# HIRO-group/torque_constrained_motion_planning

Measured on AMD Instinct MI355X. Metric: torque-feasible collision-checked RRT* samples/sec, Panda 7-DOF, 1/2/4/8 GPU, higher is better.
Workload: dtype f64

## Files before the change

include/tcmp.h:

```cpp
#ifndef TCMP_H_
#define TCMP_H_

#include <stdint.h>

#ifdef __cplusplus
extern "C" {
#endif

typedef struct tcmp_handle tcmp_handle;
typedef struct tcmp_comm tcmp_comm;

#define TCMP_TORQUE_BASE 0
#define TCMP_TORQUE_NOV 1
#define TCMP_TORQUE_RNE 2
#define TCMP_TORQUE_DYN 3

#define TCMP_PLAN_OK 0
#define TCMP_PLAN_START_GOAL_COLLISION 1
#define TCMP_PLAN_NO_GOAL 2
#define TCMP_PLAN_VALIDATION_FAILED 3
#define TCMP_PLAN_MINJERK_ASSERT 4

int tcmp_create(int device, tcmp_handle** out);
int tcmp_destroy(tcmp_handle* h);
// ... 43 lines not shown

int tcmp_check_configs(tcmp_handle* h, const double* q, int64_t n, int32_t* collides);

int tcmp_check_body(tcmp_handle* h, const double* q, int64_t n, int32_t* collides);

int tcmp_base_pd(tcmp_handle* h, double* pd, int32_t n);

enum {
  TCMP_PD_CHAIN = 0, TCMP_PD_BOX32 = 1, TCMP_PD_BOX64 = 2, TCMP_PD_HULL32 = 3, TCMP_PD_HULL64 = 4,
  TCMP_PD_LOD_IN = 5, TCMP_PD_LOD_OUT = 6, TCMP_PD_FACET_AXES = 7, TCMP_PD_SPHERE_CERT = 8
};
enum { TCMP_PD_NO_PRUNE = 1, TCMP_PD_INNER_BOX = 2 };
int tcmp_debug_pair_pd(tcmp_handle* h, const int32_t* link, const double* pose,
                       const int32_t* obstacle, int64_t n, int32_t stage, int32_t flags,
                       double* pd, int32_t* info);

int tcmp_gauss_clusters(const tcmp_hulls* H, int32_t n, double* records, float* cones,
                        int32_t* cluster_off);

int tcmp_check_edges(tcmp_handle* h, const double* from, const double* to, int64_t n,
                     const double* resolutions, int32_t torque_mode, double payload_mass,
                     int32_t* n_safe, int32_t* n_steps, double* last);

typedef struct {
  int32_t max_anchors;
  int32_t passes;
} tcmp_shortcut_cfg;

typedef struct {
  int32_t status;
// ... 150 lines not shown
```

torque_constrained_motion_planning_amd/_lib.py:

```python
import ctypes
import os
import threading

import numpy as np

HERE = os.path.dirname(os.path.abspath(__file__))
LIB_PATH = os.environ.get("TCMP_LIB_PATH", os.path.join(HERE, "libtcmp.so"))

_dp = ctypes.POINTER(ctypes.c_double)
_i32p = ctypes.POINTER(ctypes.c_int32)
_i64p = ctypes.POINTER(ctypes.c_int64)
_u8p = ctypes.POINTER(ctypes.c_uint8)

TORQUE_BASE, TORQUE_NOV, TORQUE_RNE, TORQUE_DYN = 0, 1, 2, 3
PLAN_OK, PLAN_START_GOAL_COLLISION, PLAN_NO_GOAL, PLAN_VALIDATION_FAILED, PLAN_MINJERK_ASSERT = range(5)

EXPORTS = [
    "tcmp_create", "tcmp_destroy", "tcmp_last_error", "tcmp_device_count", "tcmp_version",
    "tcmp_synchronize",
    "tcmp_set_scene", "tcmp_set_meshes", "tcmp_set_mesh_lods", "tcmp_set_mesh_spheres", "tcmp_set_self_collision", "tcmp_set_timing", "tcmp_rne_batch", "tcmp_torque_ok", "tcmp_check_configs",
    "tcmp_check_body", "tcmp_base_pd",
    "tcmp_check_edges", "tcmp_nearest", "tcmp_minjerk", "tcmp_validate_traj",
    "tcmp_plan_begin", "tcmp_plan_round", "tcmp_plan_goal", "tcmp_plan_run", "tcmp_plan_finish",
    "tcmp_plan_retrace",
    "tcmp_plan_run_shared", "tcmp_plan_run_group", "tcmp_plan_run_fused", "tcmp_plan_begin_many",
    "tcmp_plan_finish_many",
    "tcmp_plan_fetch", "tcmp_plan_tree", "tcmp_plan_digest", "tcmp_plan_debug_round", "tcmp_ik", "tcmp_fk",
    "tcmp_debug_counters", "tcmp_microbench",
    "tcmp_rendezvous", "tcmp_dist_init", "tcmp_dist_destroy", "tcmp_dist_rank",
    "tcmp_dist_barrier", "tcmp_dist_allreduce", "tcmp_dist_allgather_i64", "tcmp_gather_paths",
    "tcmp_gather_layout", "tcmp_gather_pack", "tcmp_gather_unpack", "tcmp_dist_rccl_ranks",
    "tcmp_shortcut_path", "tcmp_plan_shortcut",
    "tcmp_tier0_tables", "tcmp_tier0_masks",
    "tcmp_debug_pair_pd", "tcmp_gauss_clusters",
]
(PD_CHAIN, PD_BOX32, PD_BOX64, PD_HULL32, PD_HULL64, PD_LOD_IN, PD_LOD_OUT, PD_FACET_AXES,
 PD_SPHERE_CERT) = range(9)
PD_NO_PRUNE, PD_INNER_BOX = 1, 2
TRAJ_COLS = 22
REDUCE_SUM, REDUCE_MAX = 0, 1


class PlanCfg(ctypes.Structure):
    _fields_ = [
        ("start", ctypes.c_double * 7), ("goal", ctypes.c_double * 7),
        ("weights", ctypes.c_double * 7), ("resolutions", ctypes.c_double * 7),
        ("radius", ctypes.c_double), ("goal_probability", ctypes.c_double),
        ("goal_tolerance", ctypes.c_double), ("payload_mass", ctypes.c_double),
        ("execution_time", ctypes.c_double), ("seed", ctypes.c_uint64),
# ... 138 lines not shown
        if hasattr(L, "tcmp_shortcut_path"):
            L.tcmp_shortcut_path.argtypes = [vp, _dp, ctypes.c_int64, _dp, _dp, ctypes.c_int32,
                                             ctypes.c_double, ctypes.POINTER(ShortcutCfg), _dp,
                                             ctypes.c_int64, ctypes.POINTER(ShortcutResult)]
            L.tcmp_plan_shortcut.argtypes = [vp, ctypes.POINTER(ShortcutCfg),
                                             ctypes.POINTER(ShortcutResult)]
        if hasattr(L, "tcmp_tier0_tables"):
            _f32p, _u32p = ctypes.POINTER(ctypes.c_float), ctypes.POINTER(ctypes.c_uint32)
            L.tcmp_tier0_tables.argtypes = [_dp, ctypes.c_int32, ctypes.c_int32, _f32p, _u32p, _f32p]
            L.tcmp_tier0_masks.argtypes = [_u32p, ctypes.c_int32, _f32p, _f32p, ctypes.c_int64, _u32p]
        if hasattr(L, "tcmp_debug_pair_pd"):
            L.tcmp_debug_pair_pd.argtypes = [vp, _i32p, _dp, _i32p, ctypes.c_int64, ctypes.c_int32,
                                             ctypes.c_int32, _dp, _i32p]
            L.tcmp_gauss_clusters.argtypes = [ctypes.POINTER(Hulls), ctypes.c_int32, _dp,
                                              ctypes.POINTER(ctypes.c_float), _i32p]
        _lib = L
        return L


def _d(a):
    return None if a is None else a.ctypes.data_as(_dp)


def _rows(x, name="array"):
    a = np.ascontiguousarray(np.asarray(x, dtype=np.float64))
    if a.ndim == 1:
        a = a.reshape(1, -1)
    if a.shape[-1] != 7:
        raise ValueError("%s must have 7 columns, got shape %s" % (name, a.shape))
    return a.reshape(-1, 7)
# ... 146 lines not shown
        self._check(self.L.tcmp_base_pd(self.h, _d(out) if n else None, n))
        return out

    def debug_pair_pd(self, link, pose, obstacle, stage, flags=0):
        pose = np.ascontiguousarray(np.asarray(pose, dtype=np.float64).reshape(-1, 12))
        n = len(pose)
        link = np.ascontiguousarray(np.broadcast_to(np.asarray(link, dtype=np.int32), (n,)))
        obstacle = np.ascontiguousarray(np.broadcast_to(np.asarray(obstacle, dtype=np.int32), (n,)))
        pd = np.zeros(n)
        info = np.zeros(n, dtype=np.int32)
        self._check(self.L.tcmp_debug_pair_pd(self.h, link.ctypes.data_as(_i32p), _d(pose),
                                              obstacle.ctypes.data_as(_i32p), n, int(stage),
                                              int(flags), _d(pd), info.ctypes.data_as(_i32p)))
        return pd, info

    def check_edges(self, q_from, q_to, mode, mass, resolutions=None):
        a = _rows(q_from, "from"); b = _rows(q_to, "to")
        n = len(a)
        ns = np.zeros(n, dtype=np.int32); nt = np.zeros(n, dtype=np.int32)
        last = np.zeros((n, 7))
        res = None if resolutions is None else np.ascontiguousarray(resolutions, dtype=np.float64)
        self._check(self.L.tcmp_check_edges(self.h, _d(a), _d(b), n, _d(res), int(mode),
                                            float(mass), ns.ctypes.data_as(_i32p),
                                            nt.ctypes.data_as(_i32p), _d(last)))
        return ns, nt, last

    def shortcut_path(self, waypoints, torque_mode, payload_mass, resolutions=None, weights=None,
                      max_anchors=512, passes=1):
        if not hasattr(self.L, "tcmp_shortcut_path"):
            raise TcmpError("tcmp_shortcut_path: not in this library build")
# ... 341 lines not shown
```

torque_constrained_motion_planning_amd/csrc/tcmp_device.h:

```cpp
#pragma once
#include <hip/hip_runtime.h>
#include <stdint.h>

#define TCMP_GEO_QUAL static constexpr
#include "panda_geometry.inc"
#include "panda_lod.inc"
#include "panda_spheres.inc"

namespace tcmp {

constexpr double kPen = 0.04;

constexpr double kLo[7] = {-2.8973, -1.7628, -2.8973, -3.0718, -2.8973, -0.0175, -2.8973};
constexpr double kHi[7] = {2.8973, 1.7628, 2.8973, -0.0698, 2.8973, 3.7525, 2.8973};
constexpr double kEffort[7] = {87.0, 87.0, 87.0, 87.0, 12.0, 12.0, 12.0};

constexpr double kC90 = 6.123233995736766e-17;
constexpr double kDhA[8] = {0.0, 0.0, 0.0, 0.0825, -0.0825, 0.0, 0.088, 0.0};
constexpr double kDhD[8] = {0.333, 0.0, 0.316, 0.0, 0.384, 0.0, 0.0, 0.107};
constexpr double kDhCa[8] = {1.0, kC90, kC90, kC90, kC90, kC90, kC90, 1.0};
constexpr double kDhSa[8] = {0.0, -1.0, 1.0, 1.0, -1.0, 1.0, 1.0, 0.0};

constexpr double kMass[7] = {4.970684, 0.646926, 3.228604, 3.587895, 1.225946, 1.666555,
                             7.35522e-01};
// ... 509 lines not shown
            m0 = -m0; m1 = -m1; m2 = -m2;
          }
          const double hv = m0 * va.x + m1 * va.y + m2 * va.z;
          const double pc = m0 * cl[0] + m1 * cl[1] + m2 * cl[2];
          const double rad = h[0] * fabs(m0 * A[0] + m1 * A[3] + m2 * A[6]) +
                             h[1] * fabs(m0 * A[1] + m1 * A[4] + m2 * A[7]) +
                             h[2] * fabs(m0 * A[2] + m1 * A[5] + m2 * A[8]);
          loc = fmin(loc, (hv - pc + rad) / sqrt(len2));
        }
      }
    }
  }
  return fmin(pd, wave_min(loc));
}

__device__ __forceinline__ float wave_minf(float x) {
  x = fminf(x, dpp_f<0xB1>(x));
  x = fminf(x, dpp_f<0x4E>(x));
  x = fminf(x, dpp_f<0x124>(x));
  x = fminf(x, dpp_f<0x128>(x));
  x = fminf(x, bc15_f(x));
  x = fminf(x, bc31_f(x));
  return readlane_f(x, 63);
}
__device__ __forceinline__ float wave_minf_bc(float x) {
  x = fminf(x, dpp_f<0xB1>(x));
  x = fminf(x, dpp_f<0x4E>(x));
  x = fminf(x, dpp_f<0x124>(x));
  x = fminf(x, dpp_f<0x128>(x));
  x = fminf(x, bc15_f(x));
  x = fminf(x, bc31_f(x));
  return readlane_f(x, 63);
}
__device__ __forceinline__ float wave_maxf(float x) {
  x = fmaxf(x, dpp_f<0xB1>(x));
  x = fmaxf(x, dpp_f<0x4E>(x));
  x = fmaxf(x, dpp_f<0x124>(x));
  x = fmaxf(x, dpp_f<0x128>(x));
  x = fmaxf(x, bc15_f(x));
  x = fmaxf(x, bc31_f(x));
  return readlane_f(x, 63);
}

constexpr float kExactGuard = 1e-4f;
constexpr int max_link_edges() {
  int m = 0;
  for (int l = 0; l < TCMP_NLINKS; ++l) {
    const int n = tcmp_geo_edge_off[l + 1] - tcmp_geo_edge_off[l];
    m = n > m ? n : m;
  }
  return m;
}
#ifdef TCMP_PROF_EXACT
__device__ unsigned long long g_fa_hist[32];
__device__ unsigned long long g_sb_hist[32];
__device__ unsigned long long g_pass_stats[8];
__device__ unsigned long long g_exact_stats[32];
#endif
__device__ __forceinline__ float exact_pd_wave32(int link, const Pose pose,
                                              const double* __restrict__ ob, const Geo g,
                                              bool box_pair = false) {
  const int lane = lane_id();
#ifdef TCMP_PROF_EXACT
  unsigned long long tb = clock64();
#define TCMP_BOX_CLK(i) if (box_pair) { const unsigned long long t1 = clock64(); \
    if (lane == 0) atomicAdd(&g_exact_stats[16 + (i)], t1 - tb); tb = t1; }
#else
#define TCMP_BOX_CLK(i)
#endif
  const double* R = pose.R;
  const double* p = pose.p;
  const double d[3] = {ob[0] - p[0], ob[1] - p[1], ob[2] - p[2]};
  float cl[3], A[9];
#pragma unroll
  for (int i = 0; i < 3; ++i) {
    cl[i] = (float)(R[0 + i] * d[0] + R[3 + i] * d[1] + R[6 + i] * d[2]);
// ... 5 lines not shown
  constexpr float P = (float)kPen;
  const int v0 = tcmp_geo_vert_off[link], v1 = tcmp_geo_vert_off[link + 1];
  const int f0 = tcmp_geo_plane_off[link], f1 = tcmp_geo_plane_off[link + 1];
  const int e0 = tcmp_geo_edge_off[link], e1 = tcmp_geo_edge_off[link + 1];
  float mn0 = INFINITY, mn1 = INFINITY, mn2 = INFINITY;
  float mx0 = -INFINITY, mx1 = -INFINITY, mx2 = -INFINITY;
  for (int v = v0 + lane; v < v1; v += 64) {
    const float x = g.verts32[3 * v], y = g.verts32[3 * v + 1], z = g.verts32[3 * v + 2];
    const float d0 = A[0] * x + A[3] * y + A[6] * z;
    const float d1 = A[1] * x + A[4] * y + A[7] * z;
    const float d2 = A[2] * x + A[5] * y + A[8] * z;
    mn0 = fminf(mn0, d0); mx0 = fmaxf(mx0, d0);
    mn1 = fminf(mn1, d1); mx1 = fmaxf(mx1, d1);
    mn2 = fminf(mn2, d2); mx2 = fmaxf(mx2, d2);
  }
  mn0 = wave_minf(mn0); mn1 = wave_minf(mn1); mn2 = wave_minf(mn2);
  mx0 = wave_maxf(mx0); mx1 = wave_maxf(mx1); mx2 = wave_maxf(mx2);
  float pd;
  {
    const float pc0 = A[0] * cl[0] + A[3] * cl[1] + A[6] * cl[2];
    const float pc1 = A[1] * cl[0] + A[4] * cl[1] + A[7] * cl[2];
    const float pc2 = A[2] * cl[0] + A[5] * cl[1] + A[8] * cl[2];
    pd = fminf(fminf(mx0 - pc0 + h[0], pc0 + h[0] - mn0),
               fminf(fminf(mx1 - pc1 + h[1], pc1 + h[1] - mn1),
                     fminf(mx2 - pc2 + h[2], pc2 + h[2] - mn2)));
  }
  TCMP_BOX_CLK(0);
  if (pd < P - kExactGuard) {
#ifdef TCMP_PROF_EXACT
    if (lane == 0) atomicAdd(&g_exact_stats[0], 1ull);
#endif
    return pd;
  }
  TCMP_BOX_CLK(1);
  float loc = INFINITY;
  for (int f = f0 + lane; f < f1; f += 64) {
    const float4 n = g.planes32[f];
    const float pc = n.x * cl[0] + n.y * cl[1] + n.z * cl[2];
    const float rad = h[0] * fabsf(n.x * A[0] + n.y * A[3] + n.z * A[6]) +
                      h[1] * fabsf(n.x * A[1] + n.y * A[4] + n.z * A[7]) +
                      h[2] * fabsf(n.x * A[2] + n.y * A[5] + n.z * A[8]);
    loc = fminf(loc, n.w - pc + rad);
  }
  {
    const float lf = fminf(pd, wave_minf(loc));
    TCMP_BOX_CLK(2);
    if (lf < P - kExactGuard) {
#ifdef TCMP_PROF_EXACT
      if (lane == 0) atomicAdd(&g_exact_stats[1], 1ull);
#endif
      return lf;
    }
  }
  static_assert(max_link_edges() <= 640, "pass-1 marks: 3 bits per 64-edge slice in 32");
  bool deg = false;
  unsigned sil = 0;
  for (int it = 0, base = e0; base < e1; ++it, base += 64) {
    const int e = base + lane;
    if (e < e1) {
      const ushort4 ix = g.eidx[e];
// ... 46 lines not shown
        deg = true;
      } else {
        const float ori = m0 * (n1.x + n2.x) + m1 * (n1.y + n2.y) + m2 * (n1.z + n2.z);
        const float il = rsqrtf(len2);
        deg |= fabsf(ori) * il < 1e-4f;
        if (ori < 0.f) { m0 = -m0; m1 = -m1; m2 = -m2; }
        const float hv = m0 * ax0 + m1 * ay0 + m2 * az0;
        const float pc = m0 * cl[0] + m1 * cl[1] + m2 * cl[2];
        const float rad = h[0] * fabsf(m0 * A[0] + m1 * A[3] + m2 * A[6]) +
                          h[1] * fabsf(m0 * A[1] + m1 * A[4] + m2 * A[7]) +
                          h[2] * fabsf(m0 * A[2] + m1 * A[5] + m2 * A[8]);
        loc = fminf(loc, (hv - pc + rad) * il);
      }
    }
    if (w0 + 64 < total && !__ballot(deg)) {
      const float lf = fminf(pd, wave_minf(loc));
      if (lf < P - kExactGuard) {
#ifdef TCMP_PROF_EXACT
        if (lane == 0) atomicAdd(&g_exact_stats[2], 1ull);
        if (lane == 0 && box_pair) atomicAdd(&g_exact_stats[27], 1ull);
#endif
        return lf;
      }
    }
  }
#ifdef TCMP_PROF_EXACT
  if (lane == 0) atomicAdd(&g_exact_stats[__ballot(deg) ? 3 : 2], 1ull);
#endif
  if (__ballot(deg)) return __builtin_nanf("");
  const float full = fminf(pd, wave_minf(loc));
#ifdef TCMP_PROF_EXACT
  if (lane == 0 && box_pair) atomicAdd(&g_exact_stats[full >= P ? 28 : 29], 1ull);
#endif
  TCMP_BOX_CLK(3);
  return full;
#undef TCMP_BOX_CLK
}

}
#include "tcmp_mesh.h"
namespace tcmp {

__device__ __forceinline__ float facet_axes_wave(int link, const float R[9], const float p[3], int mi,
                                                 const int* rg, const Scene sc, const Geo g) {
  const int lane = lane_id();
  const float4* LS = sc.csph + TCMP_NSPH * link;
  const float4* MS = sc.sph + TCMP_NSPH * (TCMP_NLINKS + mi);
  float best = -INFINITY, bx = 1.f, by = 0.f, bz = 0.f;
#pragma unroll
  for (int k = lane; k < TCMP_NSPH * TCMP_NSPH; k += 64) {
    const float4 t = MS[k % TCMP_NSPH];
    const float4 s = LS[k / TCMP_NSPH];
    const float dx = t.x - p[0], dy = t.y - p[1], dz = t.z - p[2];
    const float ex = R[0] * dx + R[3] * dy + R[6] * dz - s.x;
    const float ey = R[1] * dx + R[4] * dy + R[7] * dz - s.y;
    const float ez = R[2] * dx + R[5] * dy + R[8] * dz - s.z;
    const float ov = s.w + t.w - __builtin_sqrtf(ex * ex + ey * ey + ez * ez);
    if (ov > best) { best = ov; bx = ex; by = ey; bz = ez; }
  }
  {
    const float m = wave_maxf(best);
    const int L = __builtin_ctzll(__ballot(best == m));
    bx = __shfl(bx, L); by = __shfl(by, L); bz = __shfl(bz, L);
    const float l2 = bx * bx + by * by + bz * bz;
    if (!(l2 > 1e-12f)) return INFINITY;
    const float il = rsqrtf(l2);
    bx *= il; by *= il; bz *= il;
  }
  const float ax = R[0] * bx + R[1] * by + R[2] * bz;
  const float ay = R[3] * bx + R[4] * by + R[5] * bz;
  const float az = R[6] * bx + R[7] * by + R[8] * bz;
  int fm = rg[2], fl = tcmp_geo_plane_off[link];
  {
    float sm = -INFINITY, sl = -INFINITY;
    const int m1 = rg[3];
    for (int f = rg[2] + lane; f < m1; f += 64) {
      const float4 n = sc.mp32[f];
      const float v = -(n.x * ax + n.y * ay + n.z * az);
      if (v > sm) { sm = v; fm = f; }
    }
    const int l1 = tcmp_geo_plane_off[link + 1];
    for (int f = fl + lane; f < l1; f += 64) {
      const float4 n = g.planes32[f];
      const float v = n.x * bx + n.y * by + n.z * bz;
      if (v > sl) { sl = v; fl = f; }
    }
    const float mm = wave_maxf(sm), ml = wave_maxf(sl);
    fm = __builtin_amdgcn_readfirstlane(__shfl(fm, __builtin_ctzll(__ballot(sm == mm))));
    fl = __builtin_amdgcn_readfirstlane(__shfl(fl, __builtin_ctzll(__ballot(sl == ml))));
  }
  const float4 N = sc.mp32[fm];
  const float4 F = g.planes32[fl];
  const float qx = -(R[0] * N.x + R[3] * N.y + R[6] * N.z);
  const float qy = -(R[1] * N.x + R[4] * N.y + R[7] * N.z);
  const float qz = -(R[2] * N.x + R[5] * N.y + R[8] * N.z);
  const float wx = R[0] * F.x + R[1] * F.y + R[2] * F.z;
  const float wy = R[3] * F.x + R[4] * F.y + R[5] * F.z;
  const float wz = R[6] * F.x + R[7] * F.y + R[8] * F.z;
  float h = -INFINITY, gm = INFINITY;
  const int v1 = tcmp_geo_vert_off[link + 1];
  for (int v = tcmp_geo_vert_off[link] + lane; v < v1; v += 64)
    h = fmaxf(h, sc.cv32[3 * v] * qx + sc.cv32[3 * v + 1] * qy + sc.cv32[3 * v + 2] * qz);
  const int w1 = rg[1];
  for (int w = rg[0] + lane; w < w1; w += 64) {
    const float4 x = sc.mv32[w];
    gm = fminf(gm, x.x * wx + x.y * wy + x.z * wz);
  }
  h = wave_maxf(h);
  gm = wave_minf(gm);
  const float o1 = h - (p[0] * N.x + p[1] * N.y + p[2] * N.z) + N.w;
  const float o2 = F.w + (p[0] * wx + p[1] * wy + p[2] * wz) - gm;
  return fminf(o1, o2);
}

template <bool MESH>
__device__ __forceinline__ double exact_pair(int link, const Pose PL0, const double* ps,
                                             const double* ob, const Scene sc, const Geo g,
                                             float sbest = -INFINITY) {
  const int mi = MESH ? obs_mesh(ob) : -1;
  auto pose = [&]() -> Pose {
    if (!MESH) return PL0;
    __asm__ volatile("" ::: "memory");
    Pose x;
#pragma unroll
// ... 3 lines not shown
    return x;
  };
  auto pose_to_lds = [&]() {
    double* slot = wave_pose_slot(sc.wq);
    const Pose PL = pose();
    if (lane_id() == 0) {
#pragma unroll
      for (int k = 0; k < 9; ++k) slot[k] = PL.R[k];
#pragma unroll
      for (int k = 0; k < 3; ++k) slot[9 + k] = PL.p[k];
    }
    __builtin_amdgcn_wave_barrier();
    return (const double*)slot;
  };
  if (!MESH || mi < 0) {
    const float pd32 = exact_pd_wave32(link, pose(), ob, g, true);
    if (pd32 == pd32 && fabsf(pd32 - (float)kPen) > kExactGuard) return (double)pd32;
    return exact_pd_wave(link, pose_to_lds(), ob, g.verts, g.planes, g.edges);
  }
#ifdef TCMP_PROF_EXACT
#define TCMP_MESH_STAT(i) if (lane_id() == 0) atomicAdd(&g_exact_stats[i], 1ull)
  unsigned long long tclk = clock64();
#define TCMP_MESH_CLK(i) { const unsigned long long t1 = clock64(); \
    if (lane_id() == 0) atomicAdd(&g_exact_stats[16 + (i)], t1 - tclk); tclk = t1; }
#else
#define TCMP_MESH_STAT(i)
#define TCMP_MESH_CLK(i)
#endif
  constexpr float P = (float)kPen;
  const int* rg = sc.mrange + kMrange * mi;
#ifdef TCMP_PROF_EXACT
// ... 39 lines not shown
  auto inner_lod = [&]() -> float {
    const HullA32 Ai{sc.lodv3[0], sc.lodpl[0], sc.lodei[0], sc.lodev[0], tcmp_lod_in_vert_off[link],
                     tcmp_lod_in_vert_off[link + 1], tcmp_lod_in_plane_off[link],
                     tcmp_lod_in_plane_off[link + 1], tcmp_lod_in_edge_off[link],
                     tcmp_lod_in_edge_off[link + 1]};
    const HullB32 Bi{sc.lv32[0], sc.lp32[0], sc.le32[0], rg[6], rg[7], rg[8], rg[9], rg[10], rg[11],
                     sc.lcl[0], rg[22], rg[23]};
    return hull_hull_wave32<false>(Ai, Bi, R, p, P + kExactGuard);
  };
  if (inner_first) {
    const float pi = inner_lod();
    TCMP_MESH_CLK(2);
    if (pi == pi && pi > P + kExactGuard) { TCMP_MESH_STAT(6); TCMP_FA_REC(pi); return (double)pi; }
  }
  if (!inner_first) {
    const float po = exact_pd_wave32(link, pose(), ob, g);
    TCMP_MESH_CLK(0);
    if (po == po && po < P - kExactGuard) { TCMP_MESH_STAT(4); TCMP_FA_REC(po); return (double)po; }
  }
  if (rg[18] && !inner_first) {
    const HullA32 Ao{sc.lodv3[1], sc.lodpl[1], sc.lodei[1], sc.lodev[1], tcmp_lod_out_vert_off[link],
                     tcmp_lod_out_vert_off[link + 1], tcmp_lod_out_plane_off[link],
                     tcmp_lod_out_plane_off[link + 1], tcmp_lod_out_edge_off[link],
                     tcmp_lod_out_edge_off[link + 1]};
    const HullB32 Bo{sc.lv32[1], sc.lp32[1], sc.le32[1], rg[12], rg[13], rg[14], rg[15], rg[16], rg[17],
                     sc.lcl[1], rg[24], rg[25]};
    const float pl = hull_hull_wave32<false>(Ao, Bo, R, p, P - kExactGuard);
    TCMP_MESH_CLK(1);
    if (pl == pl && pl < P - kExactGuard) { TCMP_MESH_STAT(5); TCMP_FA_REC(pl); return (double)pl; }
    if (!inner_first) {
      const float pi = inner_lod();
      TCMP_MESH_CLK(2);
      if (pi == pi && pi > P + kExactGuard) { TCMP_MESH_STAT(6); TCMP_FA_REC(pi); return (double)pi; }
    }
  } else if (!inner_first) {
    const double* ib = sc.mib + 16 * mi;
    if (ib[12] > 0.0) {
      const float pi = exact_pd_wave32(link, pose(), ib, g);
      if (pi == pi && pi > P + kExactGuard) { TCMP_MESH_STAT(6); TCMP_FA_REC(pi); return (double)pi; }
    }
  }
  const HullA32 A{g.verts32, g.planes32, g.eidx, sc.geo_ev, tcmp_geo_vert_off[link],
                  tcmp_geo_vert_off[link + 1], tcmp_geo_plane_off[link],
                  tcmp_geo_plane_off[link + 1], tcmp_geo_edge_off[link], tcmp_geo_edge_off[link + 1]};
  const HullB32 B{sc.mv32, sc.mp32, sc.me32, rg[0], rg[1], rg[2], rg[3], rg[4], rg[5], sc.mcl,
                  rg[20], rg[21]};
  const float pm = hull_hull_wave32<true>(A, B, R, p, P - kExactGuard);
  TCMP_MESH_CLK(3);
  if (pm == pm && fabsf(pm - P) > kExactGuard) { TCMP_FA_REC(pm); return (double)pm; }
  TCMP_MESH_STAT(7);
  const double r64 = exact_mesh_wave(link, pose_to_lds(), mi, sc.mrange, sc.mp64, sc.mv64, sc.me64,
                                     sc.mcl, g.verts, g.planes, g.edges);
  TCMP_MESH_CLK(4);
// ... 779 lines not shown
```

torque_constrained_motion_planning_amd/csrc/tcmp_engine.hip:

```cpp
#include <hip/hip_runtime.h>
#include <hipcub/hipcub.hpp>
#include <rocprim/device/device_radix_sort.hpp>

#include <algorithm>
#include <climits>
#include <cmath>
#include <condition_variable>
#include <mutex>
#include <thread>
#include <cstddef>
#include <cstdio>
#include <cstdlib>
#include <cstring>
#include <string>
#include <vector>

#include "tcmp_device.h"
#include "../../include/tcmp.h"
#include "tcmp_dist_internal.h"

using namespace tcmp;

namespace {

// ... 566 lines not shown
}
__global__ __launch_bounds__(256) void k_rewire_scan(const PlanParams* __restrict__ Pd, DevState* st, Tree tr,
                                                     const int* rwlist, int* nbr, int* ncount) {
  rewire_scan_block(Pd, st, tr, rwlist, nbr, ncount, blockIdx.x);
}

template <bool MESH>
__device__ __forceinline__ void rewire_apply_block(const PlanParams* __restrict__ Pd, DevState* st,
                                                   const Tree& tr, const int* rwlist,
                                                   const int* nbr, const int* ncount,
                                                   const Scene& sc_g, const Geo& g_g, int blk) {
  const PlanParams P = *Pd;
  extern __shared__ double tcmp_lds[];
  Scene sc;
  Geo g;
  stage_lds<!MESH>(sc_g, g_g, tcmp_lds, sc, g);
  const long long R = st->rw_count, T = st->snap;
  const long long t = (long long)blk * blockDim.x + threadIdx.x;
  const bool act = t < R && ncount[t] > 0;
  if (__ballot(act) == 0) return;
  const long long me = act ? rwlist[t] : 0;
  double qn[7];
  double cost_new = 0;
  int cnt = 0;
  if (act) {
    load7(tr.cfg + 8 * me, qn);
    cost_new = tr.cfg[8 * me + 7];
    cnt = ncount[t];
  } else {
    for (int k = 0; k < 7; ++k) qn[k] = 0.5 * (kLo[k] + kHi[k]);
  }
  StepStats ss = {0, 0, 0};
  int c = 0;
  int prev = -1;
// ... 405 lines not shown
#pragma unroll
      for (int k = 0; k < 3; ++k) slot[9 + k] = PL.p[k];
    }
    __builtin_amdgcn_wave_barrier();
    return (const double*)slot;
  };
  const double* ob = sc.obs + 16 * o;
  const int mi = MESH ? obs_mesh(ob) : -1;
  constexpr float P = (float)kPen;
  double out = __builtin_nan("");
  int inf = 0;
  if (stage == kDbgChain) {
    out = exact_pair<MESH>(lk, PL, ps, ob, sc, g);
  } else if (stage == kDbgBox32 || stage == kDbgBox64) {
    const double* bx = (MESH && mi >= 0 && (flags & kDbgInnerBox)) ? sc.mib + 16 * mi : ob;
    if (stage == kDbgBox32) out = (double)exact_pd_wave32(lk, PL, bx, g, mi < 0);
    else out = exact_pd_wave(lk, pose_to_lds(), bx, g.verts, g.planes, g.edges);
  } else if constexpr (MESH) {
    const int* rg = sc.mrange + kMrange * mi;
    float R[9], p[3];
#pragma unroll
    for (int k = 0; k < 9; ++k) R[k] = (float)PL.R[k];
#pragma unroll
    for (int k = 0; k < 3; ++k) p[k] = (float)PL.p[k];
    const bool prune = !(flags & kDbgNoPrune);
    if (stage == kDbgHull32) {
      const HullA32 A{g.verts32, g.planes32, g.eidx, sc.geo_ev, tcmp_geo_vert_off[lk],
                      tcmp_geo_vert_off[lk + 1], tcmp_geo_plane_off[lk], tcmp_geo_plane_off[lk + 1],
                      tcmp_geo_edge_off[lk], tcmp_geo_edge_off[lk + 1]};
      const HullB32 B{sc.mv32, sc.mp32, sc.me32, rg[0], rg[1], rg[2], rg[3], rg[4], rg[5], sc.mcl,
                      rg[20], rg[21]};
// ... 16 lines not shown
      const HullB32 B{sc.lv32[x], sc.lp32[x], sc.le32[x], r[0], r[1], r[2], r[3], r[4], r[5],
                      sc.lcl[x], rg[22 + 2 * x], rg[23 + 2 * x]};
      const float stop = x ? P - kExactGuard : P + kExactGuard;
      out = (double)(prune ? hull_hull_wave32<false, true>(A, B, R, p, stop)
                           : hull_hull_wave32<false, false>(A, B, R, p, stop));
    } else if (stage == kDbgFacetAxes) {
      out = (double)facet_axes_wave(lk, R, p, mi, rg, sc, g);
    } else if (stage == kDbgSphereCert) {
      inf = sphere_cert(lk, R, p, mi, sc, g);
      out = 0.0;
    }
  }
  if (lane == 0) {
    pd[i] = out;
    info[i] = inf;
  }
}

template <int MODE>
__global__ __launch_bounds__(256) __attribute__((amdgpu_waves_per_eu(MODE == 3 ? 1 : 2))) void k_torque(const double* q, const double* qd, const double* qdd, long long n,
                         double mass, int* ok) {
  const long long i = (long long)blockIdx.x * blockDim.x + threadIdx.x;
  if (i >= n) return;
  double x[7], v[7], a[7], cq[7], sq[7];
  load7(q + 8 * i, x);
  if (qd) load7(qd + 8 * i, v); else for (int k = 0; k < 7; ++k) v[k] = 0;
  if (qdd) load7(qdd + 8 * i, a); else for (int k = 0; k < 7; ++k) a[k] = 0;
  sincos7(x, cq, sq);
  ok[i] = torque_test_m<MODE>(mass, cq, sq, v, a) ? 1 : 0;
}
// ... 1570 lines not shown
                        h->stream));
  HIPCHK(hipMemcpyAsync(h->i0.p, link, (size_t)n * sizeof(int), hipMemcpyHostToDevice, h->stream));
  HIPCHK(hipMemcpyAsync(h->i1.p, obstacle, (size_t)n * sizeof(int), hipMemcpyHostToDevice,
                        h->stream));
  hipLaunchKernelGGL(h->mesh_kernels() ? k_debug_pair_pd<true> : k_debug_pair_pd<false>,
                     dim3(grid_for(n, 4)), dim3(256), lds_bytes(h), h->stream, h->i0.p, h->s0.p,
                     h->i1.p, (int)n, (int)stage, (int)flags, h->scene(), h->geo(), h->s1.p,
                     h->i2.p);
  HIPCHK(hipGetLastError());
  HIPCHK(hipMemcpyAsync(pd, h->s1.p, (size_t)n * sizeof(double), hipMemcpyDeviceToHost, h->stream));
  HIPCHK(hipMemcpyAsync(info, h->i2.p, (size_t)n * sizeof(int), hipMemcpyDeviceToHost, h->stream));
  if (int rc_s = sync_stream(h)) return rc_s;
  return 0;
}

int tcmp_gauss_clusters(const tcmp_hulls* H, int32_t n, double* records, float* cones,
                        int32_t* cluster_off) {
  if (n < 0 || (n > 0 && (!records || !cones || !cluster_off))) return fail(-1, "bad arguments");
  if (n == 0) return 0;
  if (int rc = check_hulls(H, n, "gauss")) return rc;
  edge_records(H->verts, H->vert_off, H->planes, H->plane_off, H->edges, H->edge_off, n, records);
  std::vector<float> cl;
  cluster_off[0] = 0;
  for (int m = 0; m < n; ++m) {
    int c0, c1;
    gauss_clusters(records, H->edge_off[m], H->edge_off[m + 1], cl, &c0, &c1);
    cluster_off[m + 1] = c1;
  }
  memcpy(cones, cl.data(), cl.size() * sizeof(float));
  return 0;
// ... 1148 lines not shown
```

torque_constrained_motion_planning_amd/csrc/tcmp_mesh.h:

```cpp
#pragma once

namespace tcmp {

#ifdef TCMP_PROF_EXACT
#define TCMP_MSTAT(i) if (lane_id() == 0) atomicAdd(&g_exact_stats[i], 1ull)
__device__ unsigned long long g_full_clk[4];
#define TCMP_FCLK(i, t) if (STAT && lane_id() == 0) atomicAdd(&g_full_clk[i], clock64() - (t))
#else
#define TCMP_MSTAT(i)
#define TCMP_FCLK(i, t)
#endif

struct HullA32 {
  const float* v3;
  const float4* pl;
  const ushort4* ei;
  const float4* ev;
  int v0, v1, f0, f1, e0, e1;
};
struct HullB32 {
  const float4* v;
  const float4* pl;
  const float* er;
  int v0, v1, f0, f1, e0, e1;
// ... 76 lines not shown
    } else {
      loc = fminf(loc, facet_pass32<1, BF>(A, B, R, p, base));
      base += 64;
    }
  }
  return loc;
}

template <bool STAT, bool PRUNE = true>
__device__ __forceinline__ float hull_hull_wave32(const HullA32 A, const HullB32 B,
                                                  const float R[9], const float p[3], float stop) {
  const int lane = lane_id();
#ifdef TCMP_PROF_EXACT
  const unsigned long long tf0 = clock64();
#endif
  float pd = wave_minf(facets32<true>(A, B, R, p));
  if (pd < stop) { if (STAT) TCMP_MSTAT(8); TCMP_FCLK(0, tf0); return pd; }
  pd = fminf(pd, wave_minf(facets32<false>(A, B, R, p)));
  if (pd < stop) { if (STAT) TCMP_MSTAT(9); TCMP_FCLK(0, tf0); return pd; }
#ifdef TCMP_PROF_EXACT
  const unsigned long long te0 = clock64();
#endif
  float loc = INFINITY;
  bool deg = false;
  const int nC = B.c1 - B.c0;
  for (int base = A.e0; base < A.e1; base += 64) {
    auto a_edge = [&](int e, float& ax, float& ay, float& az, float& bx, float& by, float& bz,
                      float& ux, float& uy, float& uz, float& ex, float& ey, float& ez,
                      float& px, float& py, float& pz) {
      const ushort4 ix = A.ei[e];
      const float4 na = A.pl[ix.z], nb = A.pl[ix.w];
      ax = R[0] * na.x + R[1] * na.y + R[2] * na.z;
      ay = R[3] * na.x + R[4] * na.y + R[5] * na.z;
// ... 129 lines not shown
          for (int u = 0; u < TCMP_REC_UNROLL; ++u) {
            const float4* E4 = reinterpret_cast<const float4*>(B.er + 16 * (k + u));
            h0[u] = E4[0];
            h1[u] = E4[1];
          }
#pragma unroll
          for (int u = 0; u < TCMP_REC_UNROLL; ++u) rec(k + u, h0[u], h1[u]);
        }
#pragma unroll 1
        for (; k < r1; ++k) {
          const float4* E4 = reinterpret_cast<const float4*>(B.er + 16 * k);
          rec(k, E4[0], E4[1]);
        }
      }
      if ((w0 + 64 < total || base + 64 < A.e1) && !__ballot(deg)) {
        const float lf = fminf(pd, wave_minf(loc));
        if (lf < stop) { if (STAT) TCMP_MSTAT(10); TCMP_FCLK(0, tf0); return lf; }
      }
    }
  }
  TCMP_FCLK(1, tf0 + (clock64() - te0));
  TCMP_FCLK(2, te0);
  if (__ballot(deg)) { if (STAT) TCMP_MSTAT(13); return __builtin_nanf(""); }
  const float res = fminf(pd, wave_minf(loc));
  if (STAT) {
    if (res >= (float)kPen) { TCMP_MSTAT(11); } else { TCMP_MSTAT(12); }
  }
  return res;
}

template <bool PRUNE = true>
__device__ __noinline__ double exact_mesh_wave(int link, const double* pose, int m,
                                               const int* __restrict__ mrange,
                                               const double4* __restrict__ mp64,
                                               const double4* __restrict__ mv64,
                                               const double* __restrict__ me64,
                                               const float4* __restrict__ mcl,
                                               const double* __restrict__ gverts,
                                               const double* __restrict__ gplanes,
// ... 93 lines not shown
```

torque_constrained_motion_planning_amd/csrc/tcmp_nn.h:

```cpp
#pragma once

constexpr int kNnC = 64;
constexpr int kNnS = 64;


__global__ __launch_bounds__(256) void k_nn_rows(DevState* st, const PlanParams* __restrict__ Pd,
                                                 const double* cfg, const int* svals,
                                                 double* stree, float* srow, long long T_bound,
                                                 int* cflag, int* sflag) {
  const long long T = st->n_nodes;
  const long long p = (long long)blockIdx.x * 256 + threadIdx.x;
  if (p >= T_bound) return;
  cflag[p] = 0;
  sflag[p] = 0;
  if (p >= T) return;
  double q[7];
  const int n = svals[p];
  load7(cfg + 8 * (size_t)n, q);
  store7(stree + 8 * p, q);
  stree[8 * p + 7] = (double)n;
  float4* d32 = reinterpret_cast<float4*>(srow + 8 * p);
  d32[0] = make_float4((float)q[0], (float)q[1], (float)q[2], (float)q[3]);
  d32[1] = make_float4((float)q[4], (float)q[5], (float)q[6], 0.f);
}
// ... 86 lines not shown
}

__global__ __launch_bounds__(256) void k_nn_build_supers(DevState* st, const int* sstart,
                                                         const float* cbox, float* sbox) {
  const int nsup = st->nn_supers;
  for (long long sw = ((long long)blockIdx.x * blockDim.x + threadIdx.x) >> 6; sw < nsup;
       sw += ((long long)gridDim.x * blockDim.x) >> 6) {
  const int c0 = sstart[sw], c1 = sstart[sw + 1];
  const long long c = c0 + lane_id();
  float lo[7], hi[7];
#pragma unroll
  for (int k = 0; k < 7; ++k) {
    lo[k] = c < c1 ? cbox[16 * c + k] : INFINITY;
    hi[k] = c < c1 ? cbox[16 * c + 8 + k] : -INFINITY;
  }
#pragma unroll
  for (int k = 0; k < 7; ++k) {
    lo[k] = wave_minf(lo[k]);
    hi[k] = wave_maxf(hi[k]);
  }
  if (lane_id() == 0) {
#pragma unroll
    for (int k = 0; k < 7; ++k) {
      sbox[16 * sw + k] = lo[k];
      sbox[16 * sw + 8 + k] = hi[k];
    }
    sbox[16 * sw + 7] = __int_as_float(c0);
    sbox[16 * sw + 15] = __int_as_float(c1 - c0);
  }
  }
}

__global__ __launch_bounds__(256) void k_nn_build_blocks(DevState* st, const float* sbox,
                                                         float* bbox) {
  const int nsup = st->nn_supers;
  for (long long b = ((long long)blockIdx.x * blockDim.x + threadIdx.x) >> 6; b * 64 < nsup;
       b += ((long long)gridDim.x * blockDim.x) >> 6) {
  const long long sp = b * 64 + lane_id();
  float lo[7], hi[7];
#pragma unroll
  for (int k = 0; k < 7; ++k) {
    lo[k] = sp < nsup ? sbox[16 * sp + k] : INFINITY;
    hi[k] = sp < nsup ? sbox[16 * sp + 8 + k] : -INFINITY;
  }
#pragma unroll
  for (int k = 0; k < 7; ++k) {
    lo[k] = wave_minf(lo[k]);
    hi[k] = wave_maxf(hi[k]);
  }
  if (lane_id() == 0) {
#pragma unroll
    for (int k = 0; k < 7; ++k) {
      bbox[16 * b + k] = lo[k];
      bbox[16 * b + 8 + k] = hi[k];
    }
    bbox[16 * b + 7] = 0.f;
    bbox[16 * b + 15] = 0.f;
  }
  }
}

__global__ void k_nn_home(DevState* st, const unsigned long long* skeys,
                          const unsigned long long* ckeys, const int* cperm, const int* cid,
                          const int* sid, int nb, int* home, int* bcount) {
// ... 30 lines not shown
```

Baseline: 140.0 million.

## Use integer-key DPP wave reductions and skip LDS staging for idle blocks

Float wave min/max reductions are replaced with an order-preserving int-key version that uses integer DPP max/min and row-broadcast DPP with identity fill, and several independent reductions are interleaved for ILP. This applies in the NN box builds and in the non-mesh exact box-PD path. The mesh path keeps the float version. Separately, the rewire kernel now returns early for blocks beyond the work count or with no active threads, before staging scene data into LDS. A debug kernel and API are added to test the reductions; NaN handling differs between int keys and fminf, which is a correctness risk.

```diff
diff --git a/include/tcmp.h b/include/tcmp.h
--- a/include/tcmp.h
+++ b/include/tcmp.h
@@ -81,6 +81,8 @@
 int tcmp_debug_pair_pd(tcmp_handle* h, const int32_t* link, const double* pose,
                        const int32_t* obstacle, int64_t n, int32_t stage, int32_t flags,
                        double* pd, int32_t* info);
+
+int tcmp_debug_wave_reduce(tcmp_handle* h, const float* values, int64_t n, float* out);
 
 int tcmp_gauss_clusters(const tcmp_hulls* H, int32_t n, double* records, float* cones,
                         int32_t* cluster_off);
diff --git a/torque_constrained_motion_planning_amd/_lib.py b/torque_constrained_motion_planning_amd/_lib.py
--- a/torque_constrained_motion_planning_amd/_lib.py
+++ b/torque_constrained_motion_planning_amd/_lib.py
@@ -32,7 +32,7 @@
     "tcmp_gather_layout", "tcmp_gather_pack", "tcmp_gather_unpack", "tcmp_dist_rccl_ranks",
     "tcmp_shortcut_path", "tcmp_plan_shortcut",
     "tcmp_tier0_tables", "tcmp_tier0_masks",
-    "tcmp_debug_pair_pd", "tcmp_gauss_clusters",
+    "tcmp_debug_pair_pd", "tcmp_gauss_clusters", "tcmp_debug_wave_reduce",
 ]
 (PD_CHAIN, PD_BOX32, PD_BOX64, PD_HULL32, PD_HULL64, PD_LOD_IN, PD_LOD_OUT, PD_FACET_AXES,
  PD_SPHERE_CERT) = range(9)
@@ -201,6 +201,9 @@
                                              ctypes.c_int32, _dp, _i32p]
             L.tcmp_gauss_clusters.argtypes = [ctypes.POINTER(Hulls), ctypes.c_int32, _dp,
                                               ctypes.POINTER(ctypes.c_float), _i32p]
+        if hasattr(L, "tcmp_debug_wave_reduce"):
+            _f32p = ctypes.POINTER(ctypes.c_float)
+            L.tcmp_debug_wave_reduce.argtypes = [vp, _f32p, ctypes.c_int64, _f32p]
         _lib = L
         return L
 
@@ -377,6 +380,17 @@
                                               int(flags), _d(pd), info.ctypes.data_as(_i32p)))
         return pd, info
 
+    def debug_wave_reduce(self, values):
+        v = np.ascontiguousarray(np.asarray(values, dtype=np.float32))
+        if v.ndim != 3 or v.shape[1:] != (64, 6):
+            raise ValueError("values must be (n, 64, 6)")
+        n = len(v)
+        out = np.zeros((n, 9), dtype=np.float32)
+        f32p = ctypes.POINTER(ctypes.c_float)
+        self._check(self.L.tcmp_debug_wave_reduce(self.h, v.ctypes.data_as(f32p), n,
+                                                  out.ctypes.data_as(f32p)))
+        return out
+
     def check_edges(self, q_from, q_to, mode, mass, resolutions=None):
         a = _rows(q_from, "from"); b = _rows(q_to, "to")
         n = len(a)
diff --git a/torque_constrained_motion_planning_amd/csrc/tcmp_device.h b/torque_constrained_motion_planning_amd/csrc/tcmp_device.h
--- a/torque_constrained_motion_planning_amd/csrc/tcmp_device.h
+++ b/torque_constrained_motion_planning_amd/csrc/tcmp_device.h
@@ -547,7 +547,7 @@
   return fmin(pd, wave_min(loc));
 }
 
-__device__ __forceinline__ float wave_minf(float x) {
+__device__ __forceinline__ float wave_minf_fp(float x) {
   x = fminf(x, dpp_f<0xB1>(x));
   x = fminf(x, dpp_f<0x4E>(x));
   x = fminf(x, dpp_f<0x124>(x));
@@ -556,16 +556,7 @@
   x = fminf(x, bc31_f(x));
   return readlane_f(x, 63);
 }
-__device__ __forceinline__ float wave_minf_bc(float x) {
-  x = fminf(x, dpp_f<0xB1>(x));
-  x = fminf(x, dpp_f<0x4E>(x));
-  x = fminf(x, dpp_f<0x124>(x));
-  x = fminf(x, dpp_f<0x128>(x));
-  x = fminf(x, bc15_f(x));
-  x = fminf(x, bc31_f(x));
-  return readlane_f(x, 63);
-}
-__device__ __forceinline__ float wave_maxf(float x) {
+__device__ __forceinline__ float wave_maxf_fp(float x) {
   x = fmaxf(x, dpp_f<0xB1>(x));
   x = fmaxf(x, dpp_f<0x4E>(x));
   x = fmaxf(x, dpp_f<0x124>(x));
@@ -574,6 +565,63 @@
   x = fmaxf(x, bc31_f(x));
   return readlane_f(x, 63);
 }
+__device__ __forceinline__ int f32_key(float x) {
+  const int i = __float_as_int(x);
+  return i ^ (int)((unsigned)(i >> 31) >> 1);
+}
+__device__ __forceinline__ float key_f32(int k) {
+  return __int_as_float(k ^ (int)((unsigned)(k >> 31) >> 1));
+}
+template <bool MX, int S>
+__device__ __forceinline__ int key_step(int k) {
+  constexpr int kId = MX ? INT_MIN : INT_MAX;
+  const int o = S == 0   ? dpp_i<0xB1>(k)
+                : S == 1 ? dpp_i<0x4E>(k)
+                : S == 2 ? dpp_i<0x124>(k)
+                : S == 3 ? dpp_i<0x128>(k)
+                : S == 4 ? __builtin_amdgcn_update_dpp(kId, k, 0x142, 0xA, 0xF, false)
+                         : __builtin_amdgcn_update_dpp(kId, k, 0x143, 0xC, 0xF, false);
+  return MX ? max(k, o) : min(k, o);
+}
+template <bool MX>
+__device__ __forceinline__ float wave_reduce_f32(float x) {
+  int k = f32_key(x);
+  k = key_step<MX, 0>(k);
+  k = key_step<MX, 1>(k);
+  k = key_step<MX, 2>(k);
+  k = key_step<MX, 3>(k);
+  k = key_step<MX, 4>(k);
+  k = key_step<MX, 5>(k);
+  return key_f32(__builtin_amdgcn_readlane(k, 63));
+}
+__device__ __forceinline__ float wave_minf(float x) { return wave_reduce_f32<false>(x); }
+__device__ __forceinline__ float wave_minf_bc(float x) { return wave_reduce_f32<false>(x); }
+__device__ __forceinline__ float wave_maxf(float x) { return wave_reduce_f32<true>(x); }
+template <int NMN, int NMX>
+__device__ __forceinline__ void wave_minmaxf(float* mn, float* mx) {
+  int a[NMN > 0 ? NMN : 1], b[NMX > 0 ? NMX : 1];
+#pragma unroll
+  for (int j = 0; j < NMN; ++j) a[j] = f32_key(mn[j]);
+#pragma unroll
+  for (int j = 0; j < NMX; ++j) b[j] = f32_key(mx[j]);
+#define TCMP_KEY_STEP(S)                                                           \
+  _Pragma("unroll") for (int j = 0; j < NMN; ++j) a[j] = key_step<false, S>(a[j]); \
+  _Pragma("unroll") for (int j = 0; j < NMX; ++j) b[j] = key_step<true, S>(b[j]);
+  TCMP_KEY_STEP(0) TCMP_KEY_STEP(1) TCMP_KEY_STEP(2) TCMP_KEY_STEP(3) TCMP_KEY_STEP(4)
+  TCMP_KEY_STEP(5)
+#undef TCMP_KEY_STEP
+#pragma unroll
+  for (int j = 0; j < NMN; ++j) mn[j] = key_f32(__builtin_amdgcn_readlane(a[j], 63));
+#pragma unroll
+  for (int j = 0; j < NMX; ++j) mx[j] = key_f32(__builtin_amdgcn_readlane(b[j], 63));
+}
+__device__ __forceinline__ void wave_minmax3(float& mn0, float& mn1, float& mn2, float& mx0,
+                                             float& mx1, float& mx2) {
+  float mn[3] = {mn0, mn1, mn2}, mx[3] = {mx0, mx1, mx2};
+  wave_minmaxf<3, 3>(mn, mx);
+  mn0 = mn[0]; mn1 = mn[1]; mn2 = mn[2];
+  mx0 = mx[0]; mx1 = mx[1]; mx2 = mx[2];
+}
 
 constexpr float kExactGuard = 1e-4f;
 constexpr int max_link_edges() {
@@ -590,9 +638,11 @@
 __device__ unsigned long long g_pass_stats[8];
 __device__ unsigned long long g_exact_stats[32];
 #endif
+template <bool KEYS>
 __device__ __forceinline__ float exact_pd_wave32(int link, const Pose pose,
                                               const double* __restrict__ ob, const Geo g,
                                               bool box_pair = false) {
+  auto wminf = [](float x) { return KEYS ? wave_minf(x) : wave_minf_fp(x); };
   const int lane = lane_id();
 #ifdef TCMP_PROF_EXACT
   unsigned long long tb = clock64();
@@ -628,8 +678,12 @@
     mn1 = fminf(mn1, d1); mx1 = fmaxf(mx1, d1);
     mn2 = fminf(mn2, d2); mx2 = fmaxf(mx2, d2);
   }
-  mn0 = wave_minf(mn0); mn1 = wave_minf(mn1); mn2 = wave_minf(mn2);
-  mx0 = wave_maxf(mx0); mx1 = wave_maxf(mx1); mx2 = wave_maxf(mx2);
+  if (KEYS) {
+    wave_minmax3(mn0, mn1, mn2, mx0, mx1, mx2);
+  } else {
+    mn0 = wave_minf_fp(mn0); mn1 = wave_minf_fp(mn1); mn2 = wave_minf_fp(mn2);
+    mx0 = wave_maxf_fp(mx0); mx1 = wave_maxf_fp(mx1); mx2 = wave_maxf_fp(mx2);
+  }
   float pd;
   {
     const float pc0 = A[0] * cl[0] + A[3] * cl[1] + A[6] * cl[2];
@@ -657,7 +711,7 @@
     loc = fminf(loc, n.w - pc + rad);
   }
   {
-    const float lf = fminf(pd, wave_minf(loc));
+    const float lf = fminf(pd, wminf(loc));
     TCMP_BOX_CLK(2);
     if (lf < P - kExactGuard) {
 #ifdef TCMP_PROF_EXACT
@@ -734,7 +788,7 @@
       }
     }
     if (w0 + 64 < total && !__ballot(deg)) {
-      const float lf = fminf(pd, wave_minf(loc));
+      const float lf = fminf(pd, wminf(loc));
       if (lf < P - kExactGuard) {
 #ifdef TCMP_PROF_EXACT
         if (lane == 0) atomicAdd(&g_exact_stats[2], 1ull);
@@ -748,7 +802,7 @@
   if (lane == 0) atomicAdd(&g_exact_stats[__ballot(deg) ? 3 : 2], 1ull);
 #endif
   if (__ballot(deg)) return __builtin_nanf("");
-  const float full = fminf(pd, wave_minf(loc));
+  const float full = fminf(pd, wminf(loc));
 #ifdef TCMP_PROF_EXACT
   if (lane == 0 && box_pair) atomicAdd(&g_exact_stats[full >= P ? 28 : 29], 1ull);
 #endif
@@ -779,7 +833,7 @@
     if (ov > best) { best = ov; bx = ex; by = ey; bz = ez; }
   }
   {
-    const float m = wave_maxf(best);
+    const float m = wave_maxf_fp(best);
     const int L = __builtin_ctzll(__ballot(best == m));
     bx = __shfl(bx, L); by = __shfl(by, L); bz = __shfl(bz, L);
     const float l2 = bx * bx + by * by + bz * bz;
@@ -805,7 +859,7 @@
       const float v = n.x * bx + n.y * by + n.z * bz;
       if (v > sl) { sl = v; fl = f; }
     }
-    const float mm = wave_maxf(sm), ml = wave_maxf(sl);
+    const float mm = wave_maxf_fp(sm), ml = wave_maxf_fp(sl);
     fm = __builtin_amdgcn_readfirstlane(__shfl(fm, __builtin_ctzll(__ballot(sm == mm))));
     fl = __builtin_amdgcn_readfirstlane(__shfl(fl, __builtin_ctzll(__ballot(sl == ml))));
   }
@@ -826,8 +880,8 @@
     const float4 x = sc.mv32[w];
     gm = fminf(gm, x.x * wx + x.y * wy + x.z * wz);
   }
-  h = wave_maxf(h);
-  gm = wave_minf(gm);
+  h = wave_maxf_fp(h);
+  gm = wave_minf_fp(gm);
   const float o1 = h - (p[0] * N.x + p[1] * N.y + p[2] * N.z) + N.w;
   const float o2 = F.w + (p[0] * wx + p[1] * wy + p[2] * wz) - gm;
   return fminf(o1, o2);
@@ -861,7 +915,7 @@
     return (const double*)slot;
   };
   if (!MESH || mi < 0) {
-    const float pd32 = exact_pd_wave32(link, pose(), ob, g, true);
+    const float pd32 = exact_pd_wave32<!MESH>(link, pose(), ob, g, true);
     if (pd32 == pd32 && fabsf(pd32 - (float)kPen) > kExactGuard) return (double)pd32;
     return exact_pd_wave(link, pose_to_lds(), ob, g.verts, g.planes, g.edges);
   }
@@ -931,7 +985,7 @@
     if (pi == pi && pi > P + kExactGuard) { TCMP_MESH_STAT(6); TCMP_FA_REC(pi); return (double)pi; }
   }
   if (!inner_first) {
-    const float po = exact_pd_wave32(link, pose(), ob, g);
+    const float po = exact_pd_wave32<!MESH>(link, pose(), ob, g);
     TCMP_MESH_CLK(0);
     if (po == po && po < P - kExactGuard) { TCMP_MESH_STAT(4); TCMP_FA_REC(po); return (double)po; }
   }
@@ -953,7 +1007,7 @@
   } else if (!inner_first) {
     const double* ib = sc.mib + 16 * mi;
     if (ib[12] > 0.0) {
-      const float pi = exact_pd_wave32(link, pose(), ib, g);
+      const float pi = exact_pd_wave32<!MESH>(link, pose(), ib, g);
       if (pi == pi && pi > P + kExactGuard) { TCMP_MESH_STAT(6); TCMP_FA_REC(pi); return (double)pi; }
     }
   }
diff --git a/torque_constrained_motion_planning_amd/csrc/tcmp_engine.hip b/torque_constrained_motion_planning_amd/csrc/tcmp_engine.hip
--- a/torque_constrained_motion_planning_amd/csrc/tcmp_engine.hip
+++ b/torque_constrained_motion_planning_amd/csrc/tcmp_engine.hip
@@ -604,10 +604,12 @@
   extern __shared__ double tcmp_lds[];
   Scene sc;
   Geo g;
-  stage_lds<!MESH>(sc_g, g_g, tcmp_lds, sc, g);
   const long long R = st->rw_count, T = st->snap;
+  if ((long long)blk * blockDim.x >= R) return;
   const long long t = (long long)blk * blockDim.x + threadIdx.x;
   const bool act = t < R && ncount[t] > 0;
+  if (!__syncthreads_or(act)) return;
+  stage_lds<!MESH>(sc_g, g_g, tcmp_lds, sc, g);
   if (__ballot(act) == 0) return;
   const long long me = act ? rwlist[t] : 0;
   double qn[7];
@@ -1043,7 +1045,7 @@
     out = exact_pair<MESH>(lk, PL, ps, ob, sc, g);
   } else if (stage == kDbgBox32 || stage == kDbgBox64) {
     const double* bx = (MESH && mi >= 0 && (flags & kDbgInnerBox)) ? sc.mib + 16 * mi : ob;
-    if (stage == kDbgBox32) out = (double)exact_pd_wave32(lk, PL, bx, g, mi < 0);
+    if (stage == kDbgBox32) out = (double)exact_pd_wave32<!MESH>(lk, PL, bx, g, mi < 0);
     else out = exact_pd_wave(lk, pose_to_lds(), bx, g.verts, g.planes, g.edges);
   } else if constexpr (MESH) {
     const int* rg = sc.mrange + kMrange * mi;
@@ -1090,6 +1092,27 @@
   if (lane == 0) {
     pd[i] = out;
     info[i] = inf;
+  }
+}
+
+__global__ __launch_bounds__(256) void k_debug_wave_reduce(const float* in, int n, float* out) {
+  const int w = __builtin_amdgcn_readfirstlane((int)(blockIdx.x * 4 + (threadIdx.x >> 6)));
+  if (w >= n) return;
+  const int lane = lane_id();
+  const float* r = in + ((size_t)w * 64 + lane) * 6;
+  float v[6];
+#pragma unroll
+  for (int k = 0; k < 6; ++k) v[k] = r[k];
+  const float x = v[0];
+  wave_minmax3(v[0], v[1], v[2], v[3], v[4], v[5]);
+  const float mn = wave_minf(x), mx = wave_maxf(x), bc = wave_minf_bc(x);
+  if (lane == 0) {
+    float* o = out + 9 * (size_t)w;
+#pragma unroll
+    for (int k = 0; k < 6; ++k) o[k] = v[k];
+    o[6] = mn;
+    o[7] = mx;
+    o[8] = bc;
   }
 }
 
@@ -2690,6 +2713,26 @@
   return 0;
 }
 
+int tcmp_debug_wave_reduce(tcmp_handle* h, const float* values, int64_t n, float* out) {
+  TCMP_ENTER(h);
+  if (n < 0 || n > (1 << 20) || (n > 0 && (!values || !out))) return fail(-1, "bad arguments");
+  if (n == 0) return 0;
+  int rc = h->s0.ensure((size_t)n * 64 * 6 / 2);
+  rc = rc ? rc : h->s1.ensure(((size_t)n * 9 + 1) / 2);
+  if (rc) return rc;
+  float* in_d = reinterpret_cast<float*>(h->s0.p);
+  float* out_d = reinterpret_cast<float*>(h->s1.p);
+  HIPCHK(hipMemcpyAsync(in_d, values, (size_t)n * 64 * 6 * sizeof(float), hipMemcpyHostToDevice,
+                        h->stream));
+  hipLaunchKernelGGL(k_debug_wave_reduce, dim3(grid_for(n, 4)), dim3(256), 0, h->stream, in_d,
+                     (int)n, out_d);
+  HIPCHK(hipGetLastError());
+  HIPCHK(hipMemcpyAsync(out, out_d, (size_t)n * 9 * sizeof(float), hipMemcpyDeviceToHost,
+                        h->stream));
+  if (int rc_s = sync_stream(h)) return rc_s;
+  return 0;
+}
+
 int tcmp_gauss_clusters(const tcmp_hulls* H, int32_t n, double* records, float* cones,
                         int32_t* cluster_off) {
   if (n < 0 || (n > 0 && (!records || !cones || !cluster_off))) return fail(-1, "bad arguments");
diff --git a/torque_constrained_motion_planning_amd/csrc/tcmp_mesh.h b/torque_constrained_motion_planning_amd/csrc/tcmp_mesh.h
--- a/torque_constrained_motion_planning_amd/csrc/tcmp_mesh.h
+++ b/torque_constrained_motion_planning_amd/csrc/tcmp_mesh.h
@@ -114,9 +114,9 @@
 #ifdef TCMP_PROF_EXACT
   const unsigned long long tf0 = clock64();
 #endif
-  float pd = wave_minf(facets32<true>(A, B, R, p));
+  float pd = wave_minf_fp(facets32<true>(A, B, R, p));
   if (pd < stop) { if (STAT) TCMP_MSTAT(8); TCMP_FCLK(0, tf0); return pd; }
-  pd = fminf(pd, wave_minf(facets32<false>(A, B, R, p)));
+  pd = fminf(pd, wave_minf_fp(facets32<false>(A, B, R, p)));
   if (pd < stop) { if (STAT) TCMP_MSTAT(9); TCMP_FCLK(0, tf0); return pd; }
 #ifdef TCMP_PROF_EXACT
   const unsigned long long te0 = clock64();
@@ -276,7 +276,7 @@
         }
       }
       if ((w0 + 64 < total || base + 64 < A.e1) && !__ballot(deg)) {
-        const float lf = fminf(pd, wave_minf(loc));
+        const float lf = fminf(pd, wave_minf_fp(loc));
         if (lf < stop) { if (STAT) TCMP_MSTAT(10); TCMP_FCLK(0, tf0); return lf; }
       }
     }
@@ -284,7 +284,7 @@
   TCMP_FCLK(1, tf0 + (clock64() - te0));
   TCMP_FCLK(2, te0);
   if (__ballot(deg)) { if (STAT) TCMP_MSTAT(13); return __builtin_nanf(""); }
-  const float res = fminf(pd, wave_minf(loc));
+  const float res = fminf(pd, wave_minf_fp(loc));
   if (STAT) {
     if (res >= (float)kPen) { TCMP_MSTAT(11); } else { TCMP_MSTAT(12); }
   }
diff --git a/torque_constrained_motion_planning_amd/csrc/tcmp_nn.h b/torque_constrained_motion_planning_amd/csrc/tcmp_nn.h
--- a/torque_constrained_motion_planning_amd/csrc/tcmp_nn.h
+++ b/torque_constrained_motion_planning_amd/csrc/tcmp_nn.h
@@ -124,11 +124,7 @@
     lo[k] = c < c1 ? cbox[16 * c + k] : INFINITY;
     hi[k] = c < c1 ? cbox[16 * c + 8 + k] : -INFINITY;
   }
-#pragma unroll
-  for (int k = 0; k < 7; ++k) {
-    lo[k] = wave_minf(lo[k]);
-    hi[k] = wave_maxf(hi[k]);
-  }
+  wave_minmaxf<7, 7>(lo, hi);
   if (lane_id() == 0) {
 #pragma unroll
     for (int k = 0; k < 7; ++k) {
@@ -153,11 +149,7 @@
     lo[k] = sp < nsup ? sbox[16 * sp + k] : INFINITY;
     hi[k] = sp < nsup ? sbox[16 * sp + 8 + k] : -INFINITY;
   }
-#pragma unroll
-  for (int k = 0; k < 7; ++k) {
-    lo[k] = wave_minf(lo[k]);
-    hi[k] = wave_maxf(hi[k]);
-  }
+  wave_minmaxf<7, 7>(lo, hi);
   if (lane_id() == 0) {
 #pragma unroll
     for (int k = 0; k < 7; ++k) {
```

New measurement: 142.2 million (median of 6 runs). 1.02x the previous value.
